# utiasSTARS/pyslam

Hardware: AMD Instinct MI355X
Metric: ms/LM-iter (Jac build + J^T J + Schur solve), stereo BA @ 500k residuals (lower is better)
Workload: dtype f64

## Files before the change

pyslam_amd/csrc/ps_abi_problem.h:

```cpp


const char* ps_last_error(void) { return g_err.c_str(); }

int ps_device_count(void) {
    int n = 0;
    if (hipGetDeviceCount(&n) != hipSuccess) return 0;
    return n;
}

int ps_warm_up(void) {
    static std::once_flag once;
    static int rc = 0;
    std::call_once(once, [] {
        void* p = nullptr;
        if (hipMalloc(&p, 256) != hipSuccess) { rc = fail("hipMalloc failed (no usable HIP device?)"); return; }
        hipLaunchKernelGGL(k_zero4, dim3(1), dim3(256), 0, 0, (size_t)8, (double*)p, (size_t)0, (double*)nullptr, (size_t)0,
                           (double*)nullptr, (size_t)0, (double*)nullptr);
        double hostw[4] = {0, 0, 0, 0};
        (void)hipMemsetAsync(p, 0, 256, 0);
        (void)hipMemcpyAsync((char*)p + 128, p, 64, hipMemcpyDeviceToDevice, 0);
        (void)hipMemcpyAsync(hostw, p, sizeof(hostw), hipMemcpyDeviceToHost, 0);
        if (hipDeviceSynchronize() != hipSuccess) rc = fail("the warm-up launch failed");
        hipFree(p);
        hipFuncAttributes a;
#define PS_TOUCH(...) (void)hipFuncGetAttributes(&a, reinterpret_cast<const void*>(&__VA_ARGS__))
        PS_TOUCH(k_landmark_pass<false>); PS_TOUCH(k_landmark_pass_packed<false, false>); PS_TOUCH(k_landmark_pass_packed<false, true>); PS_TOUCH(k_backsub_packed<false>); PS_TOUCH(k_pose_pass<false>); PS_TOUCH(k_pose_finalize); PS_TOUCH(k_schur_pairs_db<0>);
        PS_TOUCH(k_schur_combine); PS_TOUCH(k_backsub<false>); PS_TOUCH(k_cost_reproj<false>); PS_TOUCH(k_cost_packed<false>); PS_TOUCH(k_reduce3); PS_TOUCH(k_reduce_partials);
        PS_TOUCH(k_copy2); PS_TOUCH(k_zero4); PS_TOUCH(k_lag_status_check);
        PS_TOUCH(k_block_jacobi_factor<6>); PS_TOUCH(k_scale_blocks<6>); PS_TOUCH(k_scale_blocks_p<6>); PS_TOUCH(k_rows_setup<6>);
        PS_TOUCH(k_coarse_rowsums<6>); PS_TOUCH(k_coarse_matrix<6>); PS_TOUCH(k_coarse_chol<6, true>); PS_TOUCH(k_coarse_border<6>);
        PS_TOUCH(k_coarse_mreduce<6>); PS_TOUCH(k_coarse_xbuild<6>); PS_TOUCH(k_coarse_recover<6>); PS_TOUCH(k_cg_fused_lds<6, 8>);
        PS_TOUCH(k_cg_fused<6, 8>); PS_TOUCH(k_cg_unscale<6>); PS_TOUCH(k_update_poses<6>); PS_TOUCH(k_update_points);
        PS_TOUCH(k_xcoarse_rowsums<6>); PS_TOUCH(k_xcoarse_matrix<6>); PS_TOUCH(k_band_chol<6>); PS_TOUCH(k_band_inverse); PS_TOUCH(k_band_inverse_rl<false>);
        PS_TOUCH(k_band_inverse_rl<true>); PS_TOUCH(k_bp_v); PS_TOUCH(k_bp_t); PS_TOUCH(k_bp_w); PS_TOUCH(k_bp_dense_sep); PS_TOUCH(k_bp_dense);
        PS_TOUCH(k_xcg_restrict<6>); PS_TOUCH(k_xcg_f2_coarse<6, 3>); PS_TOUCH(k_xcg_fused1<6, 8, false>); PS_TOUCH(k_xcg_fused1<6, 0, true>);
        PS_TOUCH(k_xcg_fused1<6, 2, false>); PS_TOUCH(k_xcg_fused1<6, 6, false>);
        PS_TOUCH(k_factor_pass<6>); PS_TOUCH(k_factor_assemble<6>); PS_TOUCH(k_cost_factors<6>);
        PS_TOUCH(k_factor_pass<3>); PS_TOUCH(k_factor_assemble<3>); PS_TOUCH(k_cost_factors<3>); PS_TOUCH(k_block_jacobi_factor<3>);
        PS_TOUCH(k_update_poses<3>); PS_TOUCH(k_direct_solve<6>); PS_TOUCH(k_direct_solve<3>);
        PS_TOUCH(k_motion_only_solve<false>); PS_TOUCH(k_motion_only_iteration<false>);
        PS_TOUCH(k_pcg_spmv<6>); PS_TOUCH(k_pcg_spmv<3>); PS_TOUCH(k_ldi_init); PS_TOUCH(k_ldi_update); PS_TOUCH(k_ldi_gemm); PS_TOUCH(k_ldi_mirror);
        PS_TOUCH(k_ldi_ritz); PS_TOUCH(k_ldi_seed_prep); PS_TOUCH(k_ldi_fro_total); PS_TOUCH(k_ldi_pad_identity);
        PS_TOUCH(k_ldi_scaled_dense<6>); PS_TOUCH(k_ldi_sym_unscale<6>); PS_TOUCH(k_ldi_scaled_dense<3>); PS_TOUCH(k_ldi_sym_unscale<3>);
        PS_TOUCH(k_shard_pack<6>); PS_TOUCH(k_shard_unpack<6>); PS_TOUCH(k_publish); PS_TOUCH(k_cov_rhs); PS_TOUCH(k_triangulate<false>);
        PS_TOUCH(k_scale_blocks<3>); PS_TOUCH(k_rows_setup<3>); PS_TOUCH(k_coarse_rowsums<3>); PS_TOUCH(k_coarse_matrix<3>);
        PS_TOUCH(k_coarse_chol<3, true>); PS_TOUCH(k_coarse_border<3>); PS_TOUCH(k_coarse_mreduce<3>); PS_TOUCH(k_coarse_xbuild<3>);
        PS_TOUCH(k_coarse_recover<3>); PS_TOUCH(k_cg_fused_lds<3, 8>); PS_TOUCH(k_cg_unscale<3>);
#undef PS_TOUCH
    });
    return rc;
}

int ps_problem_destroy(ps_problem* h) {
    if (!h) return 0;
    if (h->cp_dbg) {
        long long c[8]; hipMemcpy(c, h->cp_dbg, 64, hipMemcpyDeviceToHost);
        int khz = 100000; hipDeviceGetAttribute(&khz, hipDeviceAttributeWallClockRate, 0);
        fprintf(stderr, "k_cg_persist, workgroup 0, %ld launches, us per launch: recurrences %.2f | sync %.2f | products + publish %.2f | gather %.2f "
                "(%.1f failed passes) | sync %.2f | dots + sync %.2f\n", h->cp_launches, c[0] * 1e3 / khz / h->cp_launches, c[1] * 1e3 / khz / h->cp_launches,
                c[2] * 1e3 / khz / h->cp_launches, c[3] * 1e3 / khz / h->cp_launches, (double)c[7] / h->cp_launches, c[4] * 1e3 / khz / h->cp_launches,
                c[5] * 1e3 / khz / h->cp_launches);
        hipFree(h->cp_dbg);
    }
    if (h->xp_dbg) {
        std::vector<long long> c(3 * 64 * 8); hipMemcpy(c.data(), h->xp_dbg, c.size() * 8, hipMemcpyDeviceToHost);
        int khz = 100000; hipDeviceGetAttribute(&khz, hipDeviceAttributeWallClockRate, 0);
        for (int w = 0; w < 3; ++w) {
            double ph[6] = {0, 0, 0, 0, 0, 0}; int np = 0;
            for (int p = 1; p < 64; ++p) {
                const long long* t = &c[((size_t)w * 64 + p) * 8];
                if (!t[6] || !t[4]) break;
                ph[0] += t[0] - t[6]; ph[1] += t[1] - t[0]; ph[2] += t[2] - t[1]; ph[3] += t[5] - t[2]; ph[4] += t[3] - t[5]; ph[5] += t[4] - t[3]; ++np;
            }
            const double u = 1e3 / khz / std::max(np, 1);
            fprintf(stderr, "k_xcg_persist, workgroup %s, last launch, %d passes, us per pass: t + coarse y %.2f | columns %.2f | products + publish %.2f | "
                    "first gather pass %.2f | rest of the gather %.2f | record sums + dots %.2f | sum %.2f\n", w == 0 ? "0" : (w == 1 ? "nwg/2" : "nwg-1"), np,
                    ph[0] * u, ph[1] * u, ph[2] * u, ph[3] * u, ph[4] * u, ph[5] * u, (ph[0] + ph[1] + ph[2] + ph[3] + ph[4] + ph[5]) * u);
        }
        hipFree(h->xp_dbg);
    }
    if (h->chk_sums) {
        hipDeviceSynchronize();
        fprintf(stderr, "PS_XCG_INV_SUM %p:", (void*)h);
        for (int k = 0; k < std::min(h->chk_nsum, 64); ++k) fprintf(stderr, " [%d use %016llx | side A_c %016llx -> inv %016llx]", k, h->chk_sums[3 * k], h->chk_sums[3 * k + 1], h->chk_sums[3 * k + 2]);
        fprintf(stderr, "\n");
        hipHostFree(h->chk_sums);
    }
    if (h->chk_cnt) {
        int32_t c[4] = {}; hipDeviceSynchronize(); hipMemcpy(c, h->chk_cnt, 16, hipMemcpyDeviceToHost);
        fprintf(stderr, "PS_XCG_AC_CHECK: %d comparisons, entries that differ between the side stream's assembly and the solver stream's: A_c %d, BSZ %d; A_c behind the assembly vs at the end of the side job: %d\n", c[2], c[0], c[1], c[3]);
        hipFree(h->chk_Ac_side); hipFree(h->chk_Ac); hipFree(h->chk_BSZ); hipFree(h->chk_cnt);
    }
    if (ps_env("PS_HOST_TIMING") && h->host_calls)
        fprintf(stderr, "ps_gn_iteration: %ld calls, %.1f us per call on the host, of which %.1f us waiting for the GPU (%ld waits)\n",
                h->host_calls, h->host_call_ns * 1e-3 / h->host_calls, h->host_wait_ns * 1e-3 / h->host_calls, h->host_waits);
    hipStreamSynchronize(h->stream);
    h->persist_release();
    if (h->side) hipStreamSynchronize(h->side);
    if (h->ldi_stream) hipStreamSynchronize(h->ldi_stream);
    cov_release(h);
    if (h->cov_xbuf) hipFree(h->cov_xbuf);
    if (h->tri_buf) hipFree(h->tri_buf);
    for (void* p : h->allocs) hipFree(p);
    h->arena_release();
    for (hipEvent_t e : h->ev_pool) hipEventDestroy(e);
    if (h->ev_ldi) { hipEventDestroy(h->ev_ldi); hipEventDestroy(h->ev_ldi_sread); }
    if (h->ldi_stream && !ps_pool().give(ps_pool().side_streams, h->ldi_stream)) hipStreamDestroy(h->ldi_stream);
    if (h->side) { hipStreamSynchronize(h->side); if (!h->side_poolable || !ps_pool().give(ps_pool().side_streams, h->side)) hipStreamDestroy(h->side); hipEventDestroy(h->ev_ac); hipEventDestroy(h->ev_chol); hipEventDestroy(h->ev_acdone); }
    if (h->own_stream && h->stream && !ps_pool().give(ps_pool().streams, h->stream)) hipStreamDestroy(h->stream);
    delete h;
    return 0;
}

struct DescStage {
    ps_problem_desc d;
    std::vector<std::vector<char>> bufs;
    int pull_bytes(const void** field, size_t bytes) {
        if (!bytes || !*field) return 0;
        bufs.emplace_back(bytes);
        if (hipMemcpy(bufs.back().data(), *field, bytes, hipMemcpyDeviceToHost) != hipSuccess)
            return fail("ps_problem_create: copy of a device-resident table failed (PS_DESC_DEVICE_TABLES set on a host pointer?)");
        *field = bufs.back().data();
        return 0;
    }
    int pull(const double** f, size_t n) { return pull_bytes((const void**)f, n * sizeof(double)); }
    int pull(const int32_t** f, size_t n) { return pull_bytes((const void**)f, n * sizeof(int32_t)); }
    bool obs_pending = false;
    int pull_obs() {
        if (!obs_pending) return 0;
        obs_pending = false;
        const size_t N = (size_t)std::max<int64_t>(0, d.num_obs);
        return pull(&d.obs_pose, N) || pull(&d.obs_point, N) || pull(&d.obs_uvd, 3 * N) || pull(&d.obs_grp, N);
    }
    int stage(const ps_problem_desc* in) {
        d = *in;
        if (!(d.flags & PS_DESC_DEVICE_TABLES)) return 0;
        const size_t P = std::max(0, d.num_poses), L = std::max(0, d.num_points), N = (size_t)std::max<int64_t>(0, d.num_obs);
        const size_t E = (size_t)std::max<int64_t>(0, d.num_edges), Q = (size_t)std::max<int64_t>(0, d.num_priors);
        const size_t X = (size_t)std::max<int64_t>(0, d.num_extra_pairs), PW = d.dof == 6 ? 12 : 6, DD = (size_t)d.dof * d.dof;
        obs_pending = N > 0;
        return pull(&d.pose_rid, P) || pull(&d.point_vid, L) || pull(&d.cams, 5 * (size_t)std::max(0, d.num_cams)) || pull(&d.stiff3, 9 * (size_t)std::max(0, d.num_stiff3)) ||
               pull(&d.obs_groups, 4 * (size_t)std::max(0, d.num_obs_groups)) || pull(&d.e_i, E) || pull(&d.e_j, E) ||
               pull(&d.e_Tobs_inv, PW * E) || pull(&d.e_grp, E) || pull(&d.u_i, Q) || pull(&d.u_Tobs_inv, PW * Q) || pull(&d.u_grp, Q) ||
               pull(&d.stiffd, DD * (size_t)std::max(0, d.num_stiffd)) || pull(&d.edge_groups, 3 * (size_t)std::max(0, d.num_edge_groups)) ||
// ... 737 lines not shown
```

pyslam_amd/csrc/ps_host_cg.h:

```cpp

namespace {

struct StageTimer {
    ps_problem* h;
    int stage;
    hipEvent_t a = nullptr, b = nullptr;
    int slot = -1;
    StageTimer(ps_problem* h_, int st, int level = 2) : h(h_), stage(st) {
        if (h->profiling < level) return;
        if (h->profiling == 1 && h->prof_every > 1 &&
            h->prof_tick % h->prof_every != (st == PS_ST_CG_KERNEL ? h->prof_every / 2 : 0)) return;
        if (h->ev_used + 2 > h->ev_pool.size()) {
            for (int i = 0; i < 64; ++i) { hipEvent_t e; hipEventCreate(&e); h->ev_pool.push_back(e); }
        }
        slot = (int)h->ev_used;
        a = h->ev_pool[h->ev_used++];
        b = h->ev_pool[h->ev_used++];
        hipEventRecord(a, h->stream);
    }
    void stop() {
        if (!a) return;
        hipEventRecord(b, h->stream);
        h->pending.push_back({stage, slot});
        a = nullptr;
// ... 251 lines not shown
    const bool split = nr > h->cg_split_min_rows;
    h->cg_split = split && !h->cg_explicit;
    for (int q = 0; q < ncb && !split; ++q) {
        for (int i = 0; i < nr; ++i) aci.push_back(i);
        for (int q2 = 0; q2 < ncb; ++q2) aci.push_back(nr + q2);
        arp[nr + q + 1] = (int32_t)aci.size();
    }
    if (split) arp.resize(nr + 1);
    if (split && !h->cg_explicit) {
        if (h->alloc(&h->cg_U, (size_t)ncb * nr * D) || h->alloc(&h->cg_cgd[0], 2 * (size_t)ncb) ||
            h->alloc(&h->cg_cgd[1], 2 * (size_t)ncb) || h->alloc(&h->cg_ab, 2)) return -1;
    }
    lap("nodes + augmented pattern");
    std::vector<int32_t> rlo, rhi, eptr, eq, elo, ehi;
    if (h->cg_explicit) eptr.assign(nr + 1, 0); else { rlo.resize((size_t)nr * ncb); rhi.resize((size_t)nr * ncb); }
    h->max_row_ents = 0;
    for (int i = 0; i < nr; ++i) {
        int lo = rp[i], hi = rp[i];
        const int end = rp[i + 1];
        const int q_first = (h->cg_explicit && end > rp[i]) ? pnode[ci[rp[i]]] : 0;
        const int q_last = (h->cg_explicit && end > rp[i]) ? std::min(ncb - 1, pnode[ci[end - 1]] + 1) : ncb - 1;
        for (int q = q_first; q <= q_last; ++q) {
            while (lo < end && ci[lo] < slo[q]) ++lo;
            while (hi < end && ci[hi] < shi[q]) ++hi;
            if (!h->cg_explicit) {
                rlo[(size_t)i * ncb + q] = arp[i] + (lo - rp[i]);
                rhi[(size_t)i * ncb + q] = arp[i] + (hi - rp[i]);
            } else if (lo < hi) {
                eq.push_back(q); elo.push_back(arp[i] + (lo - rp[i])); ehi.push_back(arp[i] + (hi - rp[i]));
            }
        }
        if (h->cg_explicit) {
            eptr[i + 1] = (int32_t)eq.size();
            h->max_row_ents = std::max(h->max_row_ents, eptr[i + 1] - eptr[i]);
        }
    }
    if (h->cg_explicit) {
        std::vector<int32_t> sptr((size_t)ncb * ncb + 1, 0), sent, srow;
        for (int q = 0; q < ncb; ++q)
            for (int i = slo[q]; i < shi[q]; ++i)
                for (int e = eptr[i]; e < eptr[i + 1]; ++e) sptr[(size_t)q * ncb + eq[e] + 1]++;
        for (size_t k = 0; k < (size_t)ncb * ncb; ++k) sptr[k + 1] += sptr[k];
        sent.resize(sptr.back()); srow.resize(sptr.back());
        std::vector<int32_t> pos(sptr.begin(), sptr.end() - 1);
        for (int q = 0; q < ncb; ++q)
            for (int i = slo[q]; i < shi[q]; ++i)
                for (int e = eptr[i]; e < eptr[i + 1]; ++e) {
                    const int32_t at = pos[(size_t)q * ncb + eq[e]]++;
                    sent[at] = e; srow[at] = i;
                }
        h->ac_bw = 0;
        for (int q = 0; q < ncb; ++q)
            for (int q2 = 0; q2 < ncb; ++q2)
                if (sptr[(size_t)q * ncb + q2 + 1] > sptr[(size_t)q * ncb + q2]) h->ac_bw = std::max(h->ac_bw, std::abs(q - q2));
        if (h->ac_bw > PS_BAND_MAXB) h->ac_bw = -1;
        if (h->ac_bw < 0 && h->coarse_req < 0 && G > 255 && !h->coarse_clamped) {
            h->coarse_clamped = true; h->coarse_built = false;
            return build_coarse(h);
        }
        if (h->upload(&h->ent_ptr, eptr) || h->upload(&h->ent_q, eq) || h->upload(&h->ent_lo, elo) ||
            h->upload(&h->ent_hi, ehi) || h->upload(&h->seg_ptr, sptr) || h->upload(&h->seg_ent, sent) ||
            h->upload(&h->seg_row, srow)) return -1;
    }
    lap("runs");
    h->ncb = ncb; h->nc = ncb * D; h->nr_aug = nr + ncb; h->nnzb_aug = (int)aci.size();
    if (h->upload(&h->pnode, pnode) || h->upload(&h->slo, slo) || h->upload(&h->shi, shi) ||
        h->upload(&h->pw0, pw0) || h->upload(&h->pw1, pw1) || (!h->cg_explicit && (h->upload(&h->run_lo, rlo) ||
        h->upload(&h->run_hi, rhi))) || h->upload(&h->arow_ptr, arp) || h->upload(&h->acol_idx, aci) ||
        h->upload(&h->aug_slot, slot) || h->upload(&h->fine_nnz, fnz)) return -1;
    lap("uploads");
    h->cp_ok = false;
    if (!h->cg_explicit && !split && (long)(nr + ncb) * D <= PS_CP_MAXN) {
        const int rows = nr + ncb;
        std::vector<CpTask> tasks;
        std::vector<int32_t> rt0(rows + 1, 0);
        for (int i = 0; i < rows; ++i) {
            rt0[i] = (int32_t)tasks.size();
            const int w = i < nr ? std::min(arp[i + 1] - arp[i], fnz[i] + ncb) : arp[i + 1] - arp[i];
            const int nt = std::max(1, cdiv(w, PS_CP_TASKB)), per = cdiv(w, nt);
            for (int k = 0; k < nt; ++k) tasks.push_back(CpTask{i, arp[i] + k * per, std::min(arp[i] + w, arp[i] + (k + 1) * per), 0});
        }
        rt0[rows] = (int32_t)tasks.size();
        const int cp_nwg = cdiv((int)tasks.size(), PS_CP_NT / 64);
        const bool cp_ne6 = (long)tasks.size() * D <= 6L * PS_CP_NT;
        int cp_per_cu = 0;
        {
            const void* kfn = D == 6 ? (cp_ne6 ? (const void*)k_cg_persist<6, 6> : (const void*)k_cg_persist<6, 12>)
                                     : (cp_ne6 ? (const void*)k_cg_persist<3, 6> : (const void*)k_cg_persist<3, 12>);
            if (hipOccupancyMaxActiveBlocksPerMultiprocessor(&cp_per_cu, kfn, PS_CP_NT, 0) != hipSuccess) { (void)hipGetLastError(); cp_per_cu = 0; }
        }
        h->cp_cus_needed = cp_per_cu > 0 ? cdiv(cp_nwg, cp_per_cu) : 0;
        if ((long)tasks.size() * D <= (long)PS_CP_NE_MAX * PS_CP_NT && h->cp_cus_needed > 0 && h->cp_cus_needed <= h->persist_capacity()) {
            CpTask* dt = nullptr;
            if (h->upload(&dt, tasks) || h->upload(&h->cp_row_task0, rt0) ||
                h->alloc(&h->cp_exch, (size_t)4 * tasks.size() * D)) return -1;
            h->cp_tasks = dt;
            HIP_OK(hipMemsetAsync(h->cp_exch, 0, (size_t)4 * tasks.size() * D * sizeof(unsigned long long), h->stream));
            h->cp_ntasks = (int)tasks.size(); h->cp_salt = 0; h->cp_ok = true;
        }
    }
    if (h->alloc(&h->BSZ, (h->cg_explicit ? eq.size() : (size_t)nr * ncb) * D * D) || h->alloc(&h->Bmat2[0], (size_t)nr * D * D) ||
        h->alloc(&h->bgv, (size_t)nr * D) || h->alloc(&h->SB, (size_t)aci.size() * D * D)) return -1;
    h->Bmat = h->Bmat2[0];
    h->lagx_ok = !h->cg_explicit && !split && h->nc <= 96 && maxlen <= PS_RS_MAXROW;
    h->side_todo = false; h->rows_attr_set = false;
    if (h->lagx_ok) {
        if (h->alloc(&h->Bmat2[1], (size_t)nr * D * D) || h->alloc(&h->X2[0], (size_t)nr * D * h->nc) ||
            h->alloc(&h->X2[1], (size_t)nr * D * h->nc) || h->alloc(&h->Mpart, (size_t)nr * h->nc * (h->nc + 1))) return -1;
        h->rows_lds = ((size_t)4 * maxlen * D * D + (size_t)D * (3 * h->nc + 1) + D * D + 3 * PS_RS_MAXROW) * sizeof(double)
                      + (PS_RS_MAXROW + 3 * 64) * sizeof(int32_t);
        h->rows_lci_lds = h->rows_lds + (size_t)h->nc * h->nc * sizeof(double) <= 160 * 1024;
        if (h->rows_lci_lds) h->rows_lds += (size_t)h->nc * h->nc * sizeof(double);
    }
    if ((!h->cg_explicit && h->alloc(&h->SZ, (size_t)nr * ncb * D * D)) || h->alloc(&h->Ac, (size_t)h->nc * h->nc) ||
        h->alloc(&h->Lci2[0], (size_t)h->nc * h->nc) || h->alloc(&h->LciT2[0], (size_t)h->nc * h->nc) ||
        h->alloc(&h->Lci2[1], (size_t)h->nc * h->nc) || h->alloc(&h->LciT2[1], (size_t)h->nc * h->nc) ||
        h->alloc(&h->tvec, (size_t)h->nc) || h->alloc(&h->chol_scratch, 2 * (size_t)h->nc * h->nc)) return -1;
    if (h->cg_explicit && (h->alloc(&h->xstate, 8) || h->alloc(&h->xy, (size_t)h->nc) || h->alloc(&h->xp2, (size_t)nr * D))) return -1;
    if (h->cg_explicit && h->ac_bw >= 0 &&
        (h->alloc(&h->Lrow, (size_t)h->nc * PS_BAND_W) || h->alloc(&h->Lcol, (size_t)h->nc * PS_BAND_W) || h->alloc(&h->rdiag, (size_t)h->nc))) return -1;
    h->xcg_rt_ok = false;
    if (h->cg_explicit && ncb <= PS_XCG_MAXNODES) {
        if (const char* e = ps_env("PS_XCG_ROWS_RT")) h->xcg_rt_rows = atoi(e);
        const int R = h->xcg_rt_rows, nwg = cdiv(nr, R);
        std::vector<int32_t> wgo((size_t)nwg * PS_XCG_NSLOT, -1), nptr(ncb + 1, 0);
        bool ok = true;
        for (int g = 0; g < nwg && ok; ++g) {
            const int first = g * R, last = std::min(nr, first + R) - 1;
            const int span = pnode[last] + 1 - pnode[first];
            if (span >= PS_XCG_NSLOT) ok = false;
            else for (int s2 = 0; s2 <= span; ++s2) nptr[pnode[first] + s2 + 1]++;
        }
        if (ok) {
            for (int q = 0; q < ncb; ++q) nptr[q + 1] += nptr[q];
            std::vector<int32_t> pos(nptr.begin(), nptr.end() - 1);
            for (int g = 0; g < nwg; ++g) {
                const int first = g * R, last = std::min(nr, first + R) - 1;
                for (int s2 = 0; s2 <= pnode[last] + 1 - pnode[first]; ++s2) wgo[(size_t)g * PS_XCG_NSLOT + s2] = pos[pnode[first] + s2]++;
            }
            if (h->upload(&h->xcg_wg_out, wgo) || h->upload(&h->xcg_nptr, nptr) ||
                h->alloc(&h->tq_part, (size_t)std::max(1, (int)nptr[ncb]) * D) || h->alloc(&h->tvec2, (size_t)h->nc)) return -1;
            h->xcg_rt_ok = true;
        }
    }
    h->xf_ok = false;
    h->xf_one_ok = h->nc <= PS_XF_NEMAX * 64 * PS_XF_ROWS && (h->nc & 1) == 0;
    if (h->cg_explicit && (h->xf_one_ok || h->nc <= PS_XF2_NEMAX * 64 * PS_XCG_CROWS_BIG) && nr >= 2 * PS_XF_ROWS) {
        const int R = PS_XF_ROWS, nwg = cdiv(nr, R);
        std::vector<int32_t> cptr(nwg + 1, 0), cols, nlo(nwg), nhi(nwg), rec((size_t)nwg * PS_XCG_NSLOT, -1), cnt(ncb, 0);
        std::vector<uint16_t> lidx((size_t)h->nnzb_aug, 0);
        std::vector<int32_t> mark(nr, -1);
        bool ok = true;
        int rmax = 1;
        for (int g = 0; g < nwg && ok; ++g) {
            const int first = g * R, last = std::min(nr, first + R) - 1;
            const size_t base = cols.size();
            for (int i = first; i <= last; ++i)
                for (int b = rp[i]; b < rp[i + 1]; ++b) if (mark[ci[b]] != g) { mark[ci[b]] = g; cols.push_back(ci[b]); }
            std::sort(cols.begin() + base, cols.end());
            const int n = (int)(cols.size() - base);
            if (n > PS_XF_CAP || n == 0) { ok = false; break; }
            cptr[g + 1] = (int32_t)cols.size();
            int lo = ncb, hi = 0;
            for (int c = 0; c < n; ++c) { const int j = cols[base + c]; lo = std::min(lo, pnode[j]); hi = std::max(hi, std::min(ncb - 1, pnode[j] + 1)); }
            if (hi - lo + 1 > PS_XF_NODES) { ok = false; break; }
            nlo[g] = lo; nhi[g] = hi;
            for (int i = first; i <= last; ++i) {
                const int a0 = arp[i];
                for (int b = rp[i]; b < rp[i + 1]; ++b)
                    lidx[slot[b]] = (uint16_t)(std::lower_bound(cols.begin() + base, cols.end(), ci[b]) - (cols.begin() + base));
                (void)a0;
            }
            const int span = pnode[last] + 1 - pnode[first];
            if (span >= PS_XCG_NSLOT) { ok = false; break; }
            for (int s2 = 0; s2 <= span; ++s2) { const int q = pnode[first] + s2; if (q < ncb) rec[(size_t)g * PS_XCG_NSLOT + s2] = cnt[q]++; }
// ... 210 lines not shown
            h->side_pending = false;
        }
        hipLaunchKernelGGL(k_coarse_rowsums<D>, dim3(nr), dim3(256), (size_t)(ncb + 1) * D * D * sizeof(double), h->stream,
                           nr, ncb, h->run_lo, h->run_hi, h->acol_idx, h->pnode, h->pw0, h->pw1, h->SB, h->SZ, h->Bmat, h->BSZ);
        hipLaunchKernelGGL(k_coarse_matrix<D>, dim3(cdiv((long)ncb * ncb * D * D, 256)), dim3(256), 0, h->stream,
                           nr, ncb, h->slo, h->shi, h->pnode, h->pw0, h->pw1, h->BSZ, h->Ac);
        auto launch_chol = [&](hipStream_t st, int buf, int32_t* stat) -> int { return coarse_factor<D>(h, st, buf, stat); };
        const bool lag = allow_lag && h->coarse_lag && h->lci_next >= 0 && (!h->cg_split || (long)h->nnzb > 24L * nr) &&
                         !(h->lagx_ok && h->lagx);
        if (lag && h->cg_split && !h->Mc && h->alloc(&h->Mc, (size_t)nc * nc)) return -1;
        h->mc_active = lag && h->cg_split;
        const int rpw = nc >= 192 ? 4 : 1;
        const int border_lds = (int)((size_t)rpw * D * nc * sizeof(double));
        if (ensure_dynamic_lds((const void*)k_coarse_border<D>, (size_t)border_lds)) return -1;
        if (lag) {
            const int use = h->lci_next;
            h->lci_cur = use;
            const CoarseRhsArgs ra{h->slo, h->shi, h->pnode, h->pw0, h->pw1, h->LciT2[use], h->tvec, h->cg_r[0], h->cg_w[0],
                                   h->cg_s[0], h->cg_p, h->cg_xh, h->cg_split ? 0 : 2, h->lag_status, h->status, h->bgv, h->cg_split ? h->Mc : nullptr};
            hipLaunchKernelGGL(k_coarse_border<D>, dim3(cdiv(nr, rpw) + ncb + 1), dim3(256), border_lds, h->stream,
                               nr, ncb, h->SZ, h->Lci2[use], h->arow_ptr, h->fine_nnz, h->Saug, h->cg_split ? 0 : 1, h->Ac, ra, rpw);
            HIP_OK(hipEventRecord(h->ev_ac, h->stream));
            HIP_OK(hipStreamWaitEvent(h->side, h->ev_ac, 0));
            if (launch_chol(h->side, use ^ 1, h->lag_status)) return -1;
            HIP_OK(hipEventRecord(h->ev_chol, h->side));
            h->lci_next = use ^ 1; h->side_pending = true;
        } else {
            const int buf = h->lci_cur;
            if (launch_chol(h->stream, buf, h->status)) return -1;
            if (h->lagx_ok)
                hipLaunchKernelGGL(k_coarse_xbuild<D>, dim3(cdiv((long)nr * D * nc, 256)), dim3(256), 0, h->stream, nr, ncb,
                                   h->pnode, h->pw0, h->pw1, h->Bmat, h->Lci2[buf], h->X2[buf]);
            const CoarseRhsArgs ra{h->slo, h->shi, h->pnode, h->pw0, h->pw1, h->LciT2[buf], h->tvec, h->cg_r[0], h->cg_w[0],
                                   h->cg_s[0], h->cg_p, h->cg_xh, h->cg_split ? 0 : 1, nullptr, h->status, h->bgv, nullptr};
            hipLaunchKernelGGL(k_coarse_border<D>, dim3(cdiv(nr, rpw) + 1), dim3(256), border_lds, h->stream,
                               nr, ncb, h->SZ, h->Lci2[buf], h->arow_ptr, h->fine_nnz, h->Saug, h->cg_split ? 0 : 1,
                               (const double*)nullptr, ra, rpw);
            h->lci_next = buf;
        }
    }
    h->cg_launched = 0;
    return 0;
}

template <int D>
int cg_side_kick(ps_problem* h) {
    if (!h->side_todo || !h->side_ready) return 0;
    h->side_todo = false;
    const int nr = h->nr, ncb = h->ncb, nc = h->nc, nb = h->side_buf;
    hipLaunchKernelGGL(k_coarse_rowsums<D>, dim3(nr), dim3(256), (size_t)(ncb + 1) * D * D * sizeof(double), h->side,
                       nr, ncb, h->run_lo, h->run_hi, h->acol_idx, h->pnode, h->pw0, h->pw1, h->SB, h->SZ, h->Bmat2[nb], h->BSZ);
    hipLaunchKernelGGL(k_coarse_matrix<D>, dim3(cdiv((long)ncb * ncb * D * D, 256)), dim3(256), 0, h->side,
                       nr, ncb, h->slo, h->shi, h->pnode, h->pw0, h->pw1, h->BSZ, h->Ac);
    if (coarse_factor<D>(h, h->side, nb, h->lag_status)) return -1;
    hipLaunchKernelGGL(k_coarse_xbuild<D>, dim3(cdiv((long)nr * D * nc, 256)), dim3(256), 0, h->side, nr, ncb,
                       h->pnode, h->pw0, h->pw1, h->Bmat2[nb], h->Lci2[nb], h->X2[nb]);
    HIP_OK(hipEventRecord(h->ev_chol, h->side));
    h->lci_next = nb; h->side_pending = true;
    return 0;
}

int side_kick(ps_problem* h) {
    if (!h->side_todo) return 0;
    return h->D == 6 ? cg_side_kick<6>(h) : cg_side_kick<3>(h);
}

template <int D>
void cg_fused_launch(ps_problem* h, double tol, int count) {
    const int cap = h->hist_cap;
    const int rows = h->cg_split ? h->nr : h->nr_aug;
    const int ncbs = h->cg_split ? h->ncb : 0;
    const double tol2 = tol * tol;
#ifdef PS_MEASURE
    if (ps_env("PS_CP_CLOCKS") && !h->cp_dbg) { hipMalloc(&h->cp_dbg, 64); hipMemset(h->cp_dbg, 0, 64); }
#endif
    if (h->cg_persist && h->cp_ok && h->G > 0 && h->cg_lds && !h->cg_split && !h->cg_two_level_reduce &&
        !h->cg_ablate && h->cg_launched == 0 && h->cg_max_launches > 0 && h->cg_max_launches <= 4090 && !h->no_repeat &&
        h->persist_reserve(h->cp_cus_needed)) {
        const int nl = h->cg_max_launches;
        if (++h->cp_salt >= (1u << 20)) {
            hipMemsetAsync(h->cp_exch, 0, (size_t)4 * h->cp_ntasks * D * sizeof(unsigned long long), h->stream);
            h->cp_salt = 1;
        }
#define PS_CP_LAUNCH(NE) hipLaunchKernelGGL((k_cg_persist<D, NE>), dim3(cdiv(h->cp_ntasks, PS_CP_NT / 64)), dim3(PS_CP_NT), 0, h->stream, h->nr_aug * D, \
                           h->cp_ntasks, (const CpTask*)h->cp_tasks, h->cp_row_task0, h->acol_idx, h->Saug, h->cg_r[0], h->cg_w[0], h->cg_s[0], h->cg_p, \
                           h->cg_xh, h->hist, cap, nl, tol2, h->status, h->scalars, h->cp_exch, h->cp_salt, h->cp_spin, h->cp_dbg,                  \
                           CpRecover{h->nr, h->ncb, h->pnode, h->pw0, h->pw1, h->Linv, h->Lci2[h->lci_cur], h->Bmat, h->x})
        if ((long)h->cp_ntasks * D <= 6L * PS_CP_NT) PS_CP_LAUNCH(6); else PS_CP_LAUNCH(12);
#undef PS_CP_LAUNCH
        h->cg_launched = nl; h->cg_kernel_launches += 1; ++h->cp_launches;
        h->cp_recovered = true;
        return;
    }
    h->cg_kernel_launches += count;
    for (int i = 0; i < count; ++i, ++h->cg_launched) {
        const int n = h->cg_launched, o = n & 1, nw = o ^ 1;
        const double* tot = h->cg_two_level_reduce ? h->cg_tot : nullptr;
        if (tot && !h->cg_split && n > 0)
            hipLaunchKernelGGL(k_cg_reduce, dim3(1), dim3(1024), 0, h->stream, rows, h->cg_gd[o], h->cg_tot, h->status);
#define PS_CG_LAUNCH(NWV)                                                                                          \
        hipLaunchKernelGGL((k_cg_fused<D, NWV>), dim3(rows), dim3(64 * NWV), 0, h->stream, rows, h->arow_ptr,           \
                           h->acol_idx, h->Saug, h->cg_r[o], h->cg_w[o], h->cg_s[o], h->cg_r[nw], h->cg_w[nw],        \
                           h->cg_s[nw], h->cg_p, h->cg_xh, h->cg_gd[o], h->cg_gd[nw], h->hist, cap, n - 1, tol2,      \
                           h->status, h->scalars, h->nr, h->ell_wf, h->ell_wc, h->cg_ablate, tot, ncbs,              \
                           h->fine_nnz, h->cg_cgd[o], h->cg_U, h->cg_ab)
        if (h->cg_lds && !h->cg_short_rows && !h->cg_split && !tot && !h->cg_ablate && rows <= 1024 &&
            (long)rows * D <= PS_CGV_MAX) {
            hipLaunchKernelGGL((k_cg_fused_lds<D, 8>), dim3(rows), dim3(512), 0, h->stream, rows, h->arow_ptr,
                               h->acol_idx, h->Saug, h->cg_r[o], h->cg_w[o], h->cg_s[o], h->cg_r[nw], h->cg_w[nw],
                               h->cg_s[nw], h->cg_p, h->cg_xh, h->cg_gd[o], h->cg_gd[nw], h->hist, cap, n - 1, tol2,
                               h->status, h->scalars, h->nr, h->ell_wf, h->ell_wc);
        }
        else if (h->cg_short_rows) { PS_CG_LAUNCH(1); }
        else if (rows > 1024) { PS_CG_LAUNCH(4); }
        else { PS_CG_LAUNCH(8); }
#undef PS_CG_LAUNCH
        if (h->cg_split)
            hipLaunchKernelGGL(k_cg_reduce_split<D>, dim3(1 + h->ncb), dim3(1024), 0, h->stream, rows, h->ncb,
                               h->cg_gd[nw], h->cg_tot, h->cg_U, h->cg_ab, h->cg_r[o], h->cg_w[o], h->cg_s[o],
                               h->cg_r[nw], h->cg_w[nw], h->cg_s[nw], h->cg_p, h->cg_xh, h->cg_cgd[nw], h->status,
                               h->mc_active ? h->Mc : (const double*)nullptr);
    }
}

template <int D>
void cg_fused_recover(ps_problem* h, const int32_t* gate) {
    const int nr = h->nr;
    if (gate && h->cp_recovered) { h->cp_recovered = false; return; }
    h->cp_recovered = false;
    if (h->G)
        hipLaunchKernelGGL(k_coarse_recover<D>, dim3(cdiv((long)nr * D, 256)), dim3(256), 0, h->stream, nr, h->ncb,
                           h->pnode, h->pw0, h->pw1, h->Linv, h->Lci2[h->lci_cur], h->cg_xh, h->x, gate, h->Bmat);
    else
        hipLaunchKernelGGL(k_cg_unscale<D>, dim3(cdiv((long)nr * D, 256)), dim3(256), 0, h->stream, nr, h->Linv,
                           h->cg_xh, h->x, gate);
}

int cg_report(ps_problem* h, int* iters_out, double* relres_out) {
    h->prev_pcg_iters = h->last_pcg_iters;
    h->last_pcg_iters = h->h_status[ST_PCG_ITERS];
    if (iters_out) *iters_out = h->h_status[ST_PCG_ITERS];
    const double rr0 = h->h_scalars[SC_RR0], rrf = h->h_scalars[SC_RRFINAL];
    if (relres_out) *relres_out = rr0 > 0.0 ? std::sqrt(rrf / rr0) : 0.0;
    if (h->h_status[ST_LM_FAIL]) {
        h->lci_next = -1;
        return fail("a landmark block H_ll is not positive definite");
    }
    if (h->h_status[ST_DIAG_FAIL]) {
        if (h->lag_status) hipMemsetAsync(h->lag_status, 0, ST_NWORDS * sizeof(int32_t), h->stream);
        h->lci_next = -1;
        return fail("reduced system has a non-positive-definite diagonal block (gauge freedom? hold a pose constant or add a prior)");
    }
    if (h->h_status[ST_PCG_DONE] == 2) {
        char buf[200];
        snprintf(buf, sizeof buf, "CG breakdown: the reduced system is not positive definite (iteration %d, relative residual %.2e)",
                 h->h_status[ST_PCG_ITERS], rr0 > 0.0 ? std::sqrt(rrf / rr0) : 0.0);
        return fail(buf);
    }
    return 0;
}

template <int D>
int cg_fused_run(ps_problem* h, double tol, int max_iters, int* iters_out, double* relres_out, bool rhs_only = false) {
    const int nvec = h->nr * D;
    double* xacc = h->q;
    double* gsaved = h->z;
    int restarts = 0, total_its = 0;
    double reduced = 1.0;
    bool rhs = rhs_only;
    for (;;) {
        const bool forced = h->cg_force_restart && restarts == 0;
        const double tol_pass = forced ? std::max(1e-4, tol) : std::min(0.1, tol / reduced);
// ... 347 lines not shown
```

pyslam_amd/csrc/ps_k_cg_persist.h:

```cpp
#pragma once

#define PS_CP_NT 512
#define PS_CP_NQ 6
#define PS_CP_TASKB (8 * PS_CP_NQ)
#define PS_CP_NV 4
#define PS_CP_NE_MAX 12
#define PS_CP_MAXN (PS_CP_NV * PS_CP_NT)
#define PS_PERSIST_TIMEOUT_TICKS 100000000LL
#ifndef PS_CP_SLEEP
#define PS_CP_SLEEP 1
#endif

struct CpTask { int32_t row, b0, b1, pad; };
struct CpRecover { int nr, ncb; const int32_t* pnode; const double *pw0, *pw1, *Linv, *Lci, *Bmat; double* x; };

typedef unsigned long long ps_u64;
typedef __attribute__((address_space(1))) ps_u64 ps_gu64;

typedef unsigned ps_u32x4 __attribute__((ext_vector_type(4)));
PS_DEV void cp_put(ps_u64* g, unsigned tag, double v) {
    const ps_u64 b = (ps_u64)__double_as_longlong(v);
    const ps_u32x4 q = {(unsigned)(b & 0xffffffffull), tag, (unsigned)(b >> 32), tag};
    asm volatile("global_store_dwordx4 %0, %1, off sc1\n\ts_nop 1" :: "v"(g), "v"(q) : "memory");
}

template <int D, int NE>
__global__ __launch_bounds__(PS_CP_NT) void k_cg_persist(
    int n , int ntasks, const CpTask* __restrict__ tasks,
    const int32_t* __restrict__ row_task0 ,
    const int32_t* __restrict__ acol_idx, const double* __restrict__ Saug,
    const double* __restrict__ r0, const double* __restrict__ w0, const double* __restrict__ s0,
    double* __restrict__ p_io, double* __restrict__ x_io,
    double* __restrict__ hist, int cap, int nlaunch , double tol2,
    int32_t* __restrict__ status, double* __restrict__ scalars,
    ps_u64* __restrict__ exch , unsigned salt, unsigned spin_limit,
    long long* __restrict__ dbg , CpRecover rec)
{
    constexpr int DD = D * D;
    __shared__ double rn[PS_CP_MAXN];
    __shared__ double wex[NE * PS_CP_NT];
    __shared__ double red[2][2][PS_CP_NT / 64];
    __shared__ int bad;
    const int t = threadIdx.x, wv = t >> 6, lane = t & 63, kk = lane >> 3, r = lane & 7;
    const int task = blockIdx.x * (PS_CP_NT / 64) + wv;
    const bool chief = blockIdx.x == 0 && t == 0;
    const size_t nex = (size_t)ntasks * D;
    if (t == 0) bad = 0;
    int b0 = 0, b1 = 0;
    if (task < ntasks) { const CpTask tk = tasks[task]; b0 = tk.b0; b1 = tk.b1; }
    int cj[PS_CP_NQ];
    double sv[PS_CP_NQ][D];
#pragma unroll
    for (int q = 0; q < PS_CP_NQ; ++q) {
        const int b = b0 + kk + 8 * q;
        cj[q] = 0;
#pragma unroll
        for (int c = 0; c < D; ++c) sv[q][c] = 0.0;
        if (b < b1 && r < D) {
            cj[q] = acol_idx[b] * D;
            const double* sb = Saug + (size_t)b * DD + r * D;
#pragma unroll
            for (int c = 0; c < D; ++c) sv[q][c] = sb[c];
        }
    }
    double vr[PS_CP_NV], vw[PS_CP_NV], vs[PS_CP_NV], vp[PS_CP_NV], vx[PS_CP_NV];
    int e0[PS_CP_NV], en[PS_CP_NV];
#pragma unroll
    for (int v = 0; v < PS_CP_NV; ++v) {
        const int i = t + v * PS_CP_NT;
        vr[v] = vw[v] = vs[v] = vp[v] = vx[v] = 0.0; e0[v] = 0; en[v] = 0;
        if (i < n) {
            vr[v] = r0[i]; vw[v] = w0[i]; vs[v] = s0[i]; vp[v] = p_io[i]; vx[v] = x_io[i];
            const int row = i / D, ta = row_task0[row];
            e0[v] = ta * D + (i - row * D); en[v] = row_task0[row + 1] - ta;
        }
    }
    if (status[ST_PCG_DONE]) return;
    double gamma = 0.0, delta = 0.0, inv_gprev = 0.0, inv_aprev = 0.0, thresh = 0.0;
    bool converged = false;
    long long ck[8] = {0, 0, 0, 0, 0, 0, 0, 0};
#define PS_CP_CLK(i) do { if (dbg) { const long long now_ = wall_clock64(); ck[i] += now_ - last_; last_ = now_; } } while (0)
    long long last_ = dbg ? wall_clock64() : 0;
    for (int k = -1; k < nlaunch - 1; ++k) {
        double alpha = 0.0, beta = 0.0;
        if (k >= 0) {
            if (k == 0) thresh = tol2 * gamma;
            if (!(gamma > thresh)) {
                if (chief) { status[ST_PCG_DONE] = (gamma != gamma) ? 2 : 1; scalars[SC_RRFINAL] = gamma; if (k == 0) scalars[SC_RR0] = gamma; }
                converged = !(gamma != gamma);
                break;
            }
            beta = (k == 0) ? 0.0 : gamma * inv_gprev;
            const double denom = (k == 0) ? delta : delta - beta * gamma * inv_aprev;
            alpha = gamma / denom;
            if (!(denom > 0.0)) {
                if (chief) { status[ST_PCG_DONE] = 2; scalars[SC_RRFINAL] = gamma; }
                break;
            }
            if (chief) {
                hist[k] = gamma; hist[cap + k] = alpha; status[ST_PCG_ITERS] = k + 1; scalars[SC_RRFINAL] = gamma;
                if (k == 0) { scalars[SC_THRESH] = thresh; scalars[SC_RR0] = gamma; }
            }
        }
        const double gamma_now = gamma, alpha_now = alpha;
        double gs = 0.0;
#pragma unroll
        for (int v = 0; v < PS_CP_NV; ++v) {
            const int i = t + v * PS_CP_NT;
            const double sn = vw[v] + beta * vs[v];
            const double pn = vr[v] + beta * vp[v];
            const double rnv = cg_rnew(vr[v], vw[v], vs[v], alpha, beta);
            vs[v] = sn; vp[v] = pn; vx[v] += alpha * pn; vr[v] = rnv;
            if (i < n) { rn[i] = rnv; gs += rnv * rnv; }
        }
        double (*rd)[PS_CP_NT / 64] = red[k & 1];
        gs = wave_sum(gs);
        if (lane == 0) rd[0][wv] = gs;
        PS_CP_CLK(0);
        __syncthreads();
        PS_CP_CLK(1);
        double gamma_next = 0.0;
#pragma unroll
        for (int w2 = 0; w2 < PS_CP_NT / 64; ++w2) gamma_next += rd[0][w2];
        const unsigned tag = salt * 4096u + (unsigned)(k + 2);
        ps_u64* buf = exch + (size_t)(k & 1) * nex * 2;
        {
            double acc = 0.0;
#pragma unroll
            for (int q = 0; q < PS_CP_NQ; ++q) {
                const double* v = rn + cj[q];
#pragma unroll
                for (int c = 0; c < D; ++c) acc += sv[q][c] * v[c];
            }
            acc += __shfl_xor(acc, 8, 64);
            acc += __shfl_xor(acc, 16, 64);
            acc += __shfl_xor(acc, 32, 64);
            if (task < ntasks && lane < D) cp_put(buf + 2 * ((size_t)task * D + lane), tag, acc);
        }
        if (k >= 0) { inv_gprev = 1.0 / gamma_now; inv_aprev = 1.0 / alpha_now; }
        PS_CP_CLK(2);
        {
            double gv[NE];
            bool ok = false;
            const long long t_enter = (long long)wall_clock64();
            for (unsigned spins = 0; !ok; ++spins) {
                ok = true;
#pragma unroll
                for (int v = 0; v < NE; ++v) {
                    const int j = t + v * PS_CP_NT;
                    gv[v] = 0.0;
                    if (j < (int)nex) {
                        const ps_u64* g = buf + 2 * (size_t)j;
                        const ps_u64 a = __hip_atomic_load((const ps_gu64*)g, __ATOMIC_RELAXED, __HIP_MEMORY_SCOPE_AGENT);
                        const ps_u64 b = __hip_atomic_load((const ps_gu64*)(g + 1), __ATOMIC_RELAXED, __HIP_MEMORY_SCOPE_AGENT);
                        ok = ok && (unsigned)(a >> 32) == tag && (unsigned)(b >> 32) == tag;
                        gv[v] = __longlong_as_double((long long)((a & 0xffffffffull) | (b << 32)));
                    }
                }
                ok = __all(ok);
                if (!ok) {
                    if (spins > spin_limit || (long long)wall_clock64() - t_enter > PS_PERSIST_TIMEOUT_TICKS) { bad = 1; break; }
                    if (PS_CP_SLEEP) __builtin_amdgcn_s_sleep(PS_CP_SLEEP);
                    ck[7] += 1;
                }
            }
#pragma unroll
            for (int v = 0; v < NE; ++v) { const int j = t + v * PS_CP_NT; if (j < (int)nex) wex[j] = gv[v]; }
        }
        PS_CP_CLK(3);
        __syncthreads();
        PS_CP_CLK(4);
#pragma unroll
        for (int v = 0; v < PS_CP_NV; ++v) {
            double wsum = 0.0;
            for (int m = 0; m < en[v]; ++m) wsum += wex[e0[v] + m * D];
            vw[v] = wsum;
        }
        double ds = 0.0;
#pragma unroll
        for (int v = 0; v < PS_CP_NV; ++v) ds += vw[v] * vr[v];
        ds = wave_sum(ds);
        if (lane == 0) rd[1][wv] = ds;
        __syncthreads();
        PS_CP_CLK(5);
        if (bad) {
            if (t == 0) { status[ST_PCG_DONE] = 2; status[ST_PERSIST_FAIL] = 1; }
            break;
        }
        gamma = gamma_next; delta = 0.0;
#pragma unroll
        for (int w2 = 0; w2 < PS_CP_NT / 64; ++w2) delta += rd[1][w2];
    }
    if (dbg && chief) for (int i = 0; i < 8; ++i) dbg[i] += ck[i];
#undef PS_CP_CLK
    if (blockIdx.x == 0) {
        if (converged && rec.x) {
            const int nc = rec.ncb * D, nf = rec.nr * D;
            __syncthreads();
#pragma unroll
            for (int v = 0; v < PS_CP_NV; ++v) { const int i = t + v * PS_CP_NT; if (i < n) rn[i] = vx[v]; }
            __syncthreads();
            const double* xc = rn + nf;
            for (int base = 0; base < nc; base += PS_CP_NT / 8) {
                const int kq = base + t / 8, sub = t & 7;
                double v = 0.0;
                if (kq < nc) for (int m = kq + sub; m < nc; m += 8) v += rec.Lci[(size_t)m * nc + kq] * xc[m];
                v += __shfl_xor(v, 1, 64); v += __shfl_xor(v, 2, 64); v += __shfl_xor(v, 4, 64);
                if (kq < nc && sub == 0) wex[kq] = v;
            }
            __syncthreads();
            for (int e = t; e < nf; e += PS_CP_NT) {
                const int i = e / D, c = e - i * D, q = rec.pnode[i];
                const double w0 = rec.pw0[i], w1 = rec.pw1[i];
                double z[D];
#pragma unroll
                for (int m = 0; m < D; ++m) z[m] = w0 * wex[q * D + m] + ((q + 1 < rec.ncb) ? w1 * wex[(q + 1) * D + m] : 0.0);
                double v = 0.0;
#pragma unroll
                for (int a = 0; a < D; ++a) {
                    double xhat = rn[i * D + a];
#pragma unroll
                    for (int m = 0; m < D; ++m) xhat += rec.Bmat[(size_t)i * DD + a * D + m] * z[m];
                    v += rec.Linv[(size_t)i * DD + a * D + c] * xhat;
                }
                rec.x[e] = v;
            }
        }
#pragma unroll
        for (int v = 0; v < PS_CP_NV; ++v) {
            const int i = t + v * PS_CP_NT;
            if (i < n) { x_io[i] = vx[v]; p_io[i] = vp[v]; }
        }
    }
}
```

Before: 0.2993.

## Gather only owned exchange entries directly in persistent CG, drop LDS staging

Each thread now loads from the global exchange buffer only the partial products it needs for its own rows, summing them in registers, instead of staging the whole exchange vector into LDS and then reducing after a barrier. This removes a __syncthreads and a large LDS array, and drops the NE template split. A convergence check before the product/publish step is also added, so the kernel can exit one pass earlier. The cost is more scattered, uncoalesced global atomic loads and extra register pressure from the unrolled prefetch of long rows.

```diff
diff --git a/pyslam_amd/csrc/ps_abi_problem.h b/pyslam_amd/csrc/ps_abi_problem.h
--- a/pyslam_amd/csrc/ps_abi_problem.h
+++ b/pyslam_amd/csrc/ps_abi_problem.h
@@ -56,10 +56,10 @@
     if (h->cp_dbg) {
         long long c[8]; hipMemcpy(c, h->cp_dbg, 64, hipMemcpyDeviceToHost);
         int khz = 100000; hipDeviceGetAttribute(&khz, hipDeviceAttributeWallClockRate, 0);
-        fprintf(stderr, "k_cg_persist, workgroup 0, %ld launches, us per launch: recurrences %.2f | sync %.2f | products + publish %.2f | gather %.2f "
-                "(%.1f failed passes) | sync %.2f | dots + sync %.2f\n", h->cp_launches, c[0] * 1e3 / khz / h->cp_launches, c[1] * 1e3 / khz / h->cp_launches,
-                c[2] * 1e3 / khz / h->cp_launches, c[3] * 1e3 / khz / h->cp_launches, (double)c[7] / h->cp_launches, c[4] * 1e3 / khz / h->cp_launches,
-                c[5] * 1e3 / khz / h->cp_launches);
+        fprintf(stderr, "k_cg_persist, workgroup 0, %ld launches, us per launch: recurrences %.2f | sync %.2f | products + publish %.2f | gather + sums %.2f "
+                "(%.1f failed passes) | dots + sync %.2f | exchanges %lld = %.2f per launch\n", h->cp_launches, c[0] * 1e3 / khz / h->cp_launches,
+                c[1] * 1e3 / khz / h->cp_launches, c[2] * 1e3 / khz / h->cp_launches, c[3] * 1e3 / khz / h->cp_launches, (double)c[7] / h->cp_launches,
+                c[5] * 1e3 / khz / h->cp_launches, c[6], (double)c[6] / h->cp_launches);
         hipFree(h->cp_dbg);
     }
     if (h->xp_dbg) {
diff --git a/pyslam_amd/csrc/ps_host_cg.h b/pyslam_amd/csrc/ps_host_cg.h
--- a/pyslam_amd/csrc/ps_host_cg.h
+++ b/pyslam_amd/csrc/ps_host_cg.h
@@ -357,15 +357,13 @@
         }
         rt0[rows] = (int32_t)tasks.size();
         const int cp_nwg = cdiv((int)tasks.size(), PS_CP_NT / 64);
-        const bool cp_ne6 = (long)tasks.size() * D <= 6L * PS_CP_NT;
         int cp_per_cu = 0;
         {
-            const void* kfn = D == 6 ? (cp_ne6 ? (const void*)k_cg_persist<6, 6> : (const void*)k_cg_persist<6, 12>)
-                                     : (cp_ne6 ? (const void*)k_cg_persist<3, 6> : (const void*)k_cg_persist<3, 12>);
+            const void* kfn = D == 6 ? (const void*)k_cg_persist<6> : (const void*)k_cg_persist<3>;
             if (hipOccupancyMaxActiveBlocksPerMultiprocessor(&cp_per_cu, kfn, PS_CP_NT, 0) != hipSuccess) { (void)hipGetLastError(); cp_per_cu = 0; }
         }
         h->cp_cus_needed = cp_per_cu > 0 ? cdiv(cp_nwg, cp_per_cu) : 0;
-        if ((long)tasks.size() * D <= (long)PS_CP_NE_MAX * PS_CP_NT && h->cp_cus_needed > 0 && h->cp_cus_needed <= h->persist_capacity()) {
+        if ((long)tasks.size() * D <= (long)PS_CP_MAXEX && h->cp_cus_needed > 0 && h->cp_cus_needed <= h->persist_capacity()) {
             CpTask* dt = nullptr;
             if (h->upload(&dt, tasks) || h->upload(&h->cp_row_task0, rt0) ||
                 h->alloc(&h->cp_exch, (size_t)4 * tasks.size() * D)) return -1;
@@ -742,12 +740,10 @@
             hipMemsetAsync(h->cp_exch, 0, (size_t)4 * h->cp_ntasks * D * sizeof(unsigned long long), h->stream);
             h->cp_salt = 1;
         }
-#define PS_CP_LAUNCH(NE) hipLaunchKernelGGL((k_cg_persist<D, NE>), dim3(cdiv(h->cp_ntasks, PS_CP_NT / 64)), dim3(PS_CP_NT), 0, h->stream, h->nr_aug * D, \
-                           h->cp_ntasks, (const CpTask*)h->cp_tasks, h->cp_row_task0, h->acol_idx, h->Saug, h->cg_r[0], h->cg_w[0], h->cg_s[0], h->cg_p, \
-                           h->cg_xh, h->hist, cap, nl, tol2, h->status, h->scalars, h->cp_exch, h->cp_salt, h->cp_spin, h->cp_dbg,                  \
-                           CpRecover{h->nr, h->ncb, h->pnode, h->pw0, h->pw1, h->Linv, h->Lci2[h->lci_cur], h->Bmat, h->x})
-        if ((long)h->cp_ntasks * D <= 6L * PS_CP_NT) PS_CP_LAUNCH(6); else PS_CP_LAUNCH(12);
-#undef PS_CP_LAUNCH
+        hipLaunchKernelGGL((k_cg_persist<D>), dim3(cdiv(h->cp_ntasks, PS_CP_NT / 64)), dim3(PS_CP_NT), 0, h->stream, h->nr_aug * D,
+                           h->cp_ntasks, (const CpTask*)h->cp_tasks, h->cp_row_task0, h->acol_idx, h->Saug, h->cg_r[0], h->cg_w[0], h->cg_s[0], h->cg_p,
+                           h->cg_xh, h->hist, cap, nl, tol2, h->status, h->scalars, h->cp_exch, h->cp_salt, h->cp_spin, h->cp_dbg,
+                           CpRecover{h->nr, h->ncb, h->pnode, h->pw0, h->pw1, h->Linv, h->Lci2[h->lci_cur], h->Bmat, h->x});
         h->cg_launched = nl; h->cg_kernel_launches += 1; ++h->cp_launches;
         h->cp_recovered = true;
         return;
diff --git a/pyslam_amd/csrc/ps_k_cg_persist.h b/pyslam_amd/csrc/ps_k_cg_persist.h
--- a/pyslam_amd/csrc/ps_k_cg_persist.h
+++ b/pyslam_amd/csrc/ps_k_cg_persist.h
@@ -4,8 +4,9 @@
 #define PS_CP_NQ 6
 #define PS_CP_TASKB (8 * PS_CP_NQ)
 #define PS_CP_NV 4
-#define PS_CP_NE_MAX 12
+#define PS_CP_MAXEX (12 * PS_CP_NT)
 #define PS_CP_MAXN (PS_CP_NV * PS_CP_NT)
+#define PS_CP_LONG 4
 #define PS_PERSIST_TIMEOUT_TICKS 100000000LL
 #ifndef PS_CP_SLEEP
 #define PS_CP_SLEEP 1
@@ -24,7 +25,11 @@
     asm volatile("global_store_dwordx4 %0, %1, off sc1\n\ts_nop 1" :: "v"(g), "v"(q) : "memory");
 }
 
-template <int D, int NE>
+PS_DEV ps_u64 cp_get(const ps_u64* buf, unsigned off) {
+    return __hip_atomic_load((const ps_gu64*)((const char*)buf + off), __ATOMIC_RELAXED, __HIP_MEMORY_SCOPE_AGENT);
+}
+
+template <int D>
 __global__ __launch_bounds__(PS_CP_NT) void k_cg_persist(
     int n , int ntasks, const CpTask* __restrict__ tasks,
     const int32_t* __restrict__ row_task0 ,
@@ -38,7 +43,7 @@
 {
     constexpr int DD = D * D;
     __shared__ double rn[PS_CP_MAXN];
-    __shared__ double wex[NE * PS_CP_NT];
+    __shared__ double yc[PS_CP_MAXN];
     __shared__ double red[2][2][PS_CP_NT / 64];
     __shared__ int bad;
     const int t = threadIdx.x, wv = t >> 6, lane = t & 63, kk = lane >> 3, r = lane & 7;
@@ -75,6 +80,9 @@
             e0[v] = ta * D + (i - row * D); en[v] = row_task0[row + 1] - ta;
         }
     }
+    int lv = -1, le0 = 0, len = 0;
+#pragma unroll
+    for (int v = PS_CP_NV - 1; v >= 0; --v) if (en[v] > 2) { lv = v; le0 = e0[v]; len = en[v]; }
     if (status[ST_PCG_DONE]) return;
     double gamma = 0.0, delta = 0.0, inv_gprev = 0.0, inv_aprev = 0.0, thresh = 0.0;
     bool converged = false;
@@ -122,6 +130,11 @@
         double gamma_next = 0.0;
 #pragma unroll
         for (int w2 = 0; w2 < PS_CP_NT / 64; ++w2) gamma_next += rd[0][w2];
+        if (k >= 0 && k + 1 < nlaunch - 1 && !(gamma_next > thresh)) {
+            if (chief) { status[ST_PCG_DONE] = (gamma_next != gamma_next) ? 2 : 1; scalars[SC_RRFINAL] = gamma_next; }
+            converged = !(gamma_next != gamma_next);
+            break;
+        }
         const unsigned tag = salt * 4096u + (unsigned)(k + 2);
         ps_u64* buf = exch + (size_t)(k & 1) * nex * 2;
         {
@@ -137,26 +150,64 @@
             acc += __shfl_xor(acc, 32, 64);
             if (task < ntasks && lane < D) cp_put(buf + 2 * ((size_t)task * D + lane), tag, acc);
         }
+        if (dbg) ck[6] += 1;
         if (k >= 0) { inv_gprev = 1.0 / gamma_now; inv_aprev = 1.0 / alpha_now; }
         PS_CP_CLK(2);
         {
-            double gv[NE];
             bool ok = false;
             const long long t_enter = (long long)wall_clock64();
             for (unsigned spins = 0; !ok; ++spins) {
                 ok = true;
-#pragma unroll
-                for (int v = 0; v < NE; ++v) {
-                    const int j = t + v * PS_CP_NT;
-                    gv[v] = 0.0;
-                    if (j < (int)nex) {
-                        const ps_u64* g = buf + 2 * (size_t)j;
-                        const ps_u64 a = __hip_atomic_load((const ps_gu64*)g, __ATOMIC_RELAXED, __HIP_MEMORY_SCOPE_AGENT);
-                        const ps_u64 b = __hip_atomic_load((const ps_gu64*)(g + 1), __ATOMIC_RELAXED, __HIP_MEMORY_SCOPE_AGENT);
-                        ok = ok && (unsigned)(a >> 32) == tag && (unsigned)(b >> 32) == tag;
-                        gv[v] = __longlong_as_double((long long)((a & 0xffffffffull) | (b << 32)));
+                ps_u64 ga[PS_CP_NV][2], gb[PS_CP_NV][2], xa[PS_CP_LONG], xb[PS_CP_LONG];
+#pragma unroll
+                for (int v = 0; v < PS_CP_NV; ++v)
+#pragma unroll
+                    for (int m = 0; m < 2; ++m) {
+                        ga[v][m] = gb[v][m] = 0;
+                        if (m < en[v]) {
+                            ga[v][m] = cp_get(buf, 16u * (unsigned)e0[v] + 16u * (m * D));
+                            gb[v][m] = cp_get(buf, 16u * (unsigned)e0[v] + 16u * (m * D) + 8u);
+                        }
                     }
-                }
+#pragma unroll
+                for (int j = 0; j < PS_CP_LONG; ++j) {
+                    xa[j] = xb[j] = 0;
+                    if (2 + j < len) {
+                        xa[j] = cp_get(buf, 16u * (unsigned)le0 + 16u * ((2 + j) * D));
+                        xb[j] = cp_get(buf, 16u * (unsigned)le0 + 16u * ((2 + j) * D) + 8u);
+                    }
+                }
+#define PS_CP_TAKE(a_, b_) do { ok = ok && (unsigned)((a_) >> 32) == tag && (unsigned)((b_) >> 32) == tag;                   \
+                                wsum += __longlong_as_double((long long)(((a_) & 0xffffffffull) | ((b_) << 32))); } while (0)
+#pragma unroll
+                for (int v = 0; v < PS_CP_NV; ++v) {
+                    double wsum = 0.0;
+#pragma unroll
+                    for (int m = 0; m < 2; ++m) if (m < en[v]) PS_CP_TAKE(ga[v][m], gb[v][m]);
+                    if (en[v] > 2) {
+                        int m0 = 2;
+                        if (v == lv) {
+#pragma unroll
+                            for (int j = 0; j < PS_CP_LONG; ++j) if (2 + j < len) PS_CP_TAKE(xa[j], xb[j]);
+                            m0 = 2 + PS_CP_LONG;
+                        }
+                        for (; m0 < en[v]; m0 += PS_CP_LONG) {
+                            ps_u64 ya[PS_CP_LONG], yb[PS_CP_LONG];
+#pragma unroll
+                            for (int j = 0; j < PS_CP_LONG; ++j) {
+                                ya[j] = yb[j] = 0;
+                                if (m0 + j < en[v]) {
+                                    ya[j] = cp_get(buf, 16u * (unsigned)(e0[v] + m0 * D) + 16u * (j * D));
+                                    yb[j] = cp_get(buf, 16u * (unsigned)(e0[v] + m0 * D) + 16u * (j * D) + 8u);
+                                }
+                            }
+#pragma unroll
+                            for (int j = 0; j < PS_CP_LONG; ++j) if (m0 + j < en[v]) PS_CP_TAKE(ya[j], yb[j]);
+                        }
+                    }
+                    vw[v] = wsum;
+                }
+#undef PS_CP_TAKE
                 ok = __all(ok);
                 if (!ok) {
                     if (spins > spin_limit || (long long)wall_clock64() - t_enter > PS_PERSIST_TIMEOUT_TICKS) { bad = 1; break; }
@@ -164,18 +215,8 @@
                     ck[7] += 1;
                 }
             }
-#pragma unroll
-            for (int v = 0; v < NE; ++v) { const int j = t + v * PS_CP_NT; if (j < (int)nex) wex[j] = gv[v]; }
         }
         PS_CP_CLK(3);
-        __syncthreads();
-        PS_CP_CLK(4);
-#pragma unroll
-        for (int v = 0; v < PS_CP_NV; ++v) {
-            double wsum = 0.0;
-            for (int m = 0; m < en[v]; ++m) wsum += wex[e0[v] + m * D];
-            vw[v] = wsum;
-        }
         double ds = 0.0;
 #pragma unroll
         for (int v = 0; v < PS_CP_NV; ++v) ds += vw[v] * vr[v];
@@ -206,7 +247,7 @@
                 double v = 0.0;
                 if (kq < nc) for (int m = kq + sub; m < nc; m += 8) v += rec.Lci[(size_t)m * nc + kq] * xc[m];
                 v += __shfl_xor(v, 1, 64); v += __shfl_xor(v, 2, 64); v += __shfl_xor(v, 4, 64);
-                if (kq < nc && sub == 0) wex[kq] = v;
+                if (kq < nc && sub == 0) yc[kq] = v;
             }
             __syncthreads();
             for (int e = t; e < nf; e += PS_CP_NT) {
@@ -214,7 +255,7 @@
                 const double w0 = rec.pw0[i], w1 = rec.pw1[i];
                 double z[D];
 #pragma unroll
-                for (int m = 0; m < D; ++m) z[m] = w0 * wex[q * D + m] + ((q + 1 < rec.ncb) ? w1 * wex[(q + 1) * D + m] : 0.0);
+                for (int m = 0; m < D; ++m) z[m] = w0 * yc[q * D + m] + ((q + 1 < rec.ncb) ? w1 * yc[(q + 1) * D + m] : 0.0);
                 double v = 0.0;
 #pragma unroll
                 for (int a = 0; a < D; ++a) {
```

Result: faster. 0.2901, median of 6 (-3.1%).
